# CLSFramework/gym-soccer-2d-env

Measured on AMD Instinct MI355X. Metric: env-steps/sec at 65536 parallel reach_ball envs per MI355X, higher is better.
Workload: dtype f32

## Files before the change

gym-soccer-2d-env_amd/csrc/s2d_device.h:

```cpp
#pragma once
#include <hip/hip_runtime.h>
#include <stdint.h>

#include "../../include/s2d.h"

#define S2D_DEV __device__ __forceinline__

enum { S2D_MODE_DISCRETE = 0, S2D_MODE_CONT1 = 1, S2D_MODE_TURN4 = 2 };

struct S2DHot {
  float inv_half_l, inv_half_w, half_l, half_w;
  float player_decay, ball_decay;
  float player_accel_max2, player_speed_max2, ball_speed_max2, rsum2;
  float stamina_max, stamina_inc_max, extra_stamina, stamina_capacity;
  float recover_init, recover_dec_thr_value, recover_min, recover_dec;
  float effort_init, effort_dec_thr_value, effort_min, effort_dec, effort_inc_thr_value, effort_inc;
  float dash_power_rate, max_dash_power, min_dash_power, max_dash_angle, min_dash_angle;
  float dash_angle_step, inv_dash_angle_step, side_dash_rate, back_dash_rate;
  float min_distance_to_ball, min_dist2_thr, act_scale;
  int max_steps, n_actions, auto_reset;
  uint32_t seed_lo, seed_hi, gid_lo, gid_hi;
  float max_moment, min_moment, inertia_moment, player_rand, ball_rand;
};
struct S2DRare {
// ... 515 lines not shown
    if (cmd == S2D_CMD_DASH) {
      dash_apply(p, e, c, ax, ay);
      accel = true;
    } else if (cmd == S2D_CMD_TURN) {
      cmd_turn(p, e, c.dir, NOISE, nz.tu);
    }
  }
  const float d2 = sim_move<NOISE>(p, rp, e, accel, ax, ay, nz);
  sim_tick_decay(p, e);
  update_stamina(p, e);
  return d2;
}

#define S2D_TAB_MAX 256
struct S2DTables { float ep[S2D_TAB_MAX], stamina[S2D_TAB_MAX], effort[S2D_TAB_MAX], recovery[S2D_TAB_MAX], capacity[S2D_TAB_MAX]; };
S2D_DEV void tables_build(const S2DHot& p, float recover_init, float cmd_power, int len, S2DTables& t) {
  Env e{};
  e.stamina = p.stamina_max; e.recovery = recover_init; e.effort = p.effort_init; e.capacity = p.stamina_capacity;
  update_stamina(p, e);
  for (int s = 0; s < len; ++s) {
    t.stamina[s] = e.stamina; t.effort[s] = e.effort; t.recovery[s] = e.recovery; t.capacity[s] = e.capacity;
    const float avail = e.stamina + p.extra_stamina;
    const float need = (cmd_power > avail) ? avail : cmd_power;
    const float st = e.stamina - need;
    t.ep[s] = e.effort * need;
    e.stamina = st > 0.0f ? st : 0.0f;
    update_stamina(p, e);
  }
}
template <bool NOISE>
// ... 177 lines not shown
```

gym-soccer-2d-env_amd/csrc/s2d_engine.hip:

```cpp
#include <hip/hip_runtime.h>

#include <cmath>
#include <cstdio>
#include <cstdlib>
#include <cstring>
#include <new>
#include <string>
#include <type_traits>

#include "s2d_device.h"

#include "s2d_actor_launch.h"
#include "s2d_kernels.h"

__global__ void s2d_tables_kernel(S2DHot p, const S2DRare* __restrict__ rp, S2DTables* __restrict__ t) {
  if (blockIdx.x == 0 && threadIdx.x == 0 && rp->tab_len > 0) tables_build(p, rp->recover_init, rp->tab_power, rp->tab_len, *t);
}
__global__ __launch_bounds__(kBlock) void s2d_init_kernel(S2DHot p, const S2DRare* __restrict__ rp,
                                                          float* __restrict__ S, int64_t stride, int64_t n) {
  int64_t i = (int64_t)blockIdx.x * kBlock + threadIdx.x;
  if (i >= n) return;
  S[F_STAMINA * stride + i] = p.stamina_max;
  S[F_RECOVERY * stride + i] = rp->recover_init;
  S[F_EFFORT * stride + i] = p.effort_init;
  S[F_CAPACITY * stride + i] = p.stamina_capacity;
}

template <int NK>
__global__ __launch_bounds__(kBlock) void s2d_reach_reset_kernel(S2DHot p, const S2DRare* __restrict__ rp,
                                                                 float* __restrict__ S, int64_t stride, int64_t n,
                                                                 const uint8_t* __restrict__ mask, StepOut o) {
// ... 230 lines not shown
  }
  store_obs_tile(lds[wv], ob, lane, active, o.obs + wave_first * S2D_OBS_DIM, valid);
  stats_store(srow, lane, sold, wave_first == 0 ? (unsigned long long)n * (unsigned long long)n_steps : 0ull, c1, c2, c3);
}

template <int MODE, int NK>
__global__ __launch_bounds__(kBlock) void s2d_reach_rollout_kernel(S2DHot p_sgpr, const S2DRare* __restrict__ rp,
                                                                   float* __restrict__ S, int64_t stride, int64_t n,
                                                                   int n_steps, const void* __restrict__ actions,
                                                                   int kind, RolloutOut ro, StepOut o) {
  constexpr bool NOISE = NK != S2D_NK_OFF;
  __shared__ __attribute__((aligned(16))) float lds[kWavesPerBlock][kObsTile];
  __shared__ PrepTile prep[kWavesPerBlock];
  __shared__ float4 act_lut[kWavesPerBlock][kWave];
  __shared__ float ep_lds[S2D_TAB_MAX];
  __shared__ float2 sc_lut[361];
  const S2DHot p = hot_in_vgprs(p_sgpr);
  const int lane = threadIdx.x & (kWave - 1), wv = threadIdx.x / kWave;
  const int64_t i = (int64_t)blockIdx.x * kBlock + threadIdx.x;
  const int64_t wave_first = i - lane;
  const S2DTables* const tb = tables_of(rp);
  const int tab_len = MODE != S2D_MODE_TURN4 ? rp->tab_len : 0;
  if (tab_len > 0) {
    for (int k = threadIdx.x; k < tab_len; k += kBlock) ep_lds[k] = tb->ep[k];
    for (int k = threadIdx.x; k <= 360; k += kBlock) {
      float sn, cs;
      sincos_deg((float)(k - 180), sn, cs);
      sc_lut[k] = make_float2(sn, cs);
    }
    __syncthreads();
  }
  if (wave_first >= n) return;
  const bool active = i < n;
  int64_t rows = n - wave_first; if (rows > kWave) rows = kWave;
  const int valid = (int)rows * S2D_OBS_DIM;
  const bool use_k = uses_policy_step<MODE, NOISE>(kind);
  uint32_t* const kplane = reinterpret_cast<uint32_t*>(S + F_POLICY * stride);
  Env e;
  uint32_t gl = 0, gh = 0, k0 = 0;
  if (active) {
    env_load(e, S, stride, i);
    if (use_k) k0 = kplane[i];
    uint64_t gid = (((uint64_t)p.gid_hi << 32) | p.gid_lo) + (uint64_t)i;
    gl = (uint32_t)gid; gh = (uint32_t)(gid >> 32);
// ... 104 lines not shown
#endif

#ifdef S2D_STAMPS
#define WS_STAMP_DECL uint64_t st_busy = 0, st_t0 = __builtin_amdgcn_s_memtime(); const uint64_t st_begin = st_t0, st_rt0 = __builtin_amdgcn_s_memrealtime()
#define WS_BARRIER() do { st_busy += __builtin_amdgcn_s_memtime() - st_t0; __syncthreads(); st_t0 = __builtin_amdgcn_s_memtime(); } while (0)
#define WS_STAMP_STORE() do { if (lane == 0) { float* q_ = o.terminal_obs + (wave_first + 2 * role) * S2D_OBS_DIM; \
    q_[0] = (float)st_busy; q_[1] = (float)(__builtin_amdgcn_s_memtime() - st_begin); q_[2] = (float)(st_rt0 & 0xffffff); \
    q_[3] = (float)(__builtin_amdgcn_s_memrealtime() & 0xffffff); \
    q_[4] = __int_as_float((int)__builtin_amdgcn_s_getreg((31 << 11) | 4)); q_[5] = __int_as_float((int)__builtin_amdgcn_s_getreg((31 << 11) | 20)); } } while (0)
#else
#define WS_STAMP_DECL do {} while (0)
#define WS_BARRIER() __syncthreads()
#define WS_STAMP_STORE() do {} while (0)
#endif

template <int MODE, int NK, int REC = 0>
__global__ __launch_bounds__(kWsBlock, 4) void s2d_reach_rollout_ws_kernel(S2DHot p_sgpr, const S2DRare* __restrict__ rp,
                                                                        float* __restrict__ S, int64_t stride,
                                                                        int64_t n, int n_steps,
                                                                        const void* __restrict__ actions, int kind,
                                                                        RolloutOut ro, StepOut o) {
  constexpr bool NOISE = NK != S2D_NK_OFF;
  constexpr int kActWords = NOISE ? (int)WA_WORDS : (int)WA_NPM;
  __shared__ float act[3][kActWords][kWave];
  __shared__ float snap[2][WS_WORDS][kWave];
  __shared__ float slots[kSlots][SL_WORDS][kWave];
  __shared__ __attribute__((aligned(16))) float tile[2][kObsTile];
  __shared__ float4 act_lut[kWave];
  __shared__ float ep_lds[S2D_TAB_MAX];
  __shared__ float2 sc_lut[361];
  const int lane = threadIdx.x & (kWave - 1);
  const int role = __builtin_amdgcn_readfirstlane(threadIdx.x / kWave);
  const bool nt = REC == 2 || (REC == 0 && ro.nt != 0);
  const int64_t wave_first = (int64_t)blockIdx.x * kWave;
  const int64_t i = wave_first + lane;
  const bool active = i < n;
  int64_t rows = n - wave_first; rows = rows > kWave ? kWave : rows;
  const int valid = (int)rows * S2D_OBS_DIM;
  const int n_iter = n_steps + 3;

  if (role != 1 && p_sgpr.auto_reset) {
    const uint64_t gid = (((uint64_t)p_sgpr.gid_hi << 32) | p_sgpr.gid_lo) + (uint64_t)i;
    uint32_t ep0 = 0u;
    if (active) ep0 = reinterpret_cast<const uint32_t*>(S + F_EPISODE * stride)[i];
    const int k = role == 0 ? 0 : role - 1;
    slot_fill_coop<NK>(p_sgpr, rp, slots[k], lane, (uint32_t)gid, (uint32_t)(gid >> 32), ep0 + 1u + (uint32_t)k, active,
                          reinterpret_cast<uint32_t*>(&tile[0][0]) + role * kWave);
  }

  if (role == 0) {
    if constexpr (NOISE) __builtin_amdgcn_s_setprio(S2D_NPRIO_P);
    const S2DHot& p = p_sgpr;
    const bool use_k = uses_policy_step<MODE, NOISE>(kind);
    uint32_t* const kplane = reinterpret_cast<uint32_t*>(S + F_POLICY * stride);
    uint32_t gl = 0, gh = 0, k0 = 0;
    if (active) {
      if (use_k) k0 = kplane[i];
      uint64_t gid = (((uint64_t)p.gid_hi << 32) | p.gid_lo) + (uint64_t)i;
      gl = (uint32_t)gid; gh = (uint32_t)(gid >> 32);
    }
    U4 quad{0, 0, 0, 0}, squad{0, 0, 0, 0}, nblk{0, 0, 0, 0};
    float dir = 0.0f; int cmd = 0;
    int64_t row = 0;
    const bool lut = MODE == S2D_MODE_DISCRETE && kind == S2D_ACT_RANDOM && p.n_actions <= kWave;
    if (lut && lane < p.n_actions) {
// ... 39 lines not shown
      wslot = wslot == 2 ? 0 : wslot + 1;
    };
    for (int s = 0; s < n_iter; ++s) {
      if (s == 0 && n_steps > 0) policy_step(0);
      if (s + 1 < n_steps) policy_step(s + 1);
      WS_BARRIER();
    }
    WS_STAMP_STORE();
    if (active) {
      if (use_k) kplane[i] = k0 + (uint32_t)n_steps;
      o.action_dir[i] = dir; o.action_cmd[i] = (uint8_t)cmd;
    }
  } else if (role == 1) {
    if constexpr (NOISE) __builtin_amdgcn_s_setprio(S2D_NPRIO_S);
    else __builtin_amdgcn_s_setprio(S2D_PRIO_S);
    const S2DHot p = hot_in_vgprs(p_sgpr);
    Env e;
    uint32_t gl = 0, gh = 0;
    int nth = 0, j = 0;
    if (active) {
      env_load(e, S, stride, i);
      uint64_t gid = (((uint64_t)p.gid_hi << 32) | p.gid_lo) + (uint64_t)i;
      gl = (uint32_t)gid; gh = (uint32_t)(gid >> 32);
      asm volatile("" ::"v"(e.px), "v"(e.py), "v"(e.vx), "v"(e.vy), "v"(e.body), "v"(e.stamina), "v"(e.effort),
                   "v"(e.recovery), "v"(e.capacity), "v"(e.bx), "v"(e.by), "v"(e.bvx), "v"(e.bvy),
                   "v"(e.step_number), "v"(e.cycle), "v"(e.episode));
    }
    const S2DTables* const tb = tables_of(rp);
    const int tab_len = MODE != S2D_MODE_TURN4 ? rp->tab_len : 0;
    bool fast = false;
    if (tab_len > 0) {
      bool ok = true;
      if (active) {
        const int sn = e.step_number;
        ok = sn >= 0 && sn < tab_len;
        const int q = ok ? sn : 0;
        ok = ok && e.stamina == tb->stamina[q] && e.effort == tb->effort[q] && e.recovery == tb->recovery[q] &&
             e.capacity == tb->capacity[q] && e.body == rintf(e.body) && fabsf(e.body) <= 180.0f;
      }
      fast = __ballot(active && !ok) == 0ull;
      if (fast)
        for (int k = lane; k < tab_len; k += kWave) ep_lds[k] = tb->ep[k];
    }
    if (fast || NK == S2D_NK_LATTICE) {
      for (int k = lane; k <= 360; k += kWave) {
        float sn, cs;
        sincos_deg((float)(k - 180), sn, cs);
        sc_lut[k] = make_float2(sn, cs);
      }
    }
    const ResetStamina rst = reset_stamina(p, rp);
    __syncthreads();
    WS_STAMP_DECL;
    auto loop = [&](auto fast_tag) {
      constexpr bool FAST = decltype(fast_tag)::value;
      struct ActRegs { float cmd, power, dir, rate, npm, nps, npc, nbm, nbs, nbc, ntu; };
      ActRegs cur{}, nxt{};
      float ep_cur = 0.0f; float2 sc_cur = make_float2(0.0f, 0.0f);
      int rslot = 1;
      auto fetch = [&](int slot) {
        ActRegs r{};
        if (MODE == S2D_MODE_TURN4) r.cmd = act[slot][WA_CMD][lane];
        if (!FAST) r.power = act[slot][WA_POWER][lane];
        r.dir = act[slot][WA_DIR][lane]; r.rate = act[slot][WA_RATE][lane];
// ... 174 lines not shown
        if ((fw & 0xff) && auto_reset) {
          const float (*sl)[kWave] = slots[fw >> 8];
#pragma unroll
          for (int k = 4; k < S2D_OBS_DIM; ++k) term_row[k] = ob6[k];
#pragma unroll
          for (int k = 4; k < S2D_OBS_DIM; ++k) ob6[k] = sl[SL_FIRST + k][lane];
        }
        if (REC != 0 || ro.obs) {
          float* t = &tile[b][lane * S2D_OBS_DIM];
#pragma unroll
          for (int k = 4; k < S2D_OBS_DIM; ++k) t[k] = ob6[k];
        }
      }
      WS_BARRIER();
    };
    {
      int s = 0;
      for (; s < 3 && s < n_iter; ++s) ball_iteration(s, std::false_type{});
      for (; s < n_steps + 2; ++s) ball_iteration(s, std::true_type{});
      for (; s < n_iter; ++s) ball_iteration(s, std::false_type{});
    }
    WS_STAMP_STORE();
    if (active) {
#pragma unroll
      for (int k = 4; k < S2D_OBS_DIM; ++k) o.obs[i * S2D_OBS_DIM + k] = ob6[k];
    }
  }
}

__global__ __launch_bounds__(kBlock) void s2d_world_model_kernel(const float* __restrict__ S, int64_t stride,
                                                                 int64_t n, S2DWorldModel w) {
// ... 149 lines not shown
                                     int64_t n, int n_steps, const void* actions_dev, int kind, const RolloutOut* ro,
                                     const StepOut* o, void* stream, char* name);


struct S2DEngine {
  S2DConfig cfg;
  S2DHot hot;
  S2DRare rare;
  const S2DRare* rare_dev;
  int mode;
  bool noise;
  int nk;
  int rollout_ws;
  int rollout_e;
  int rollout_nt;
  char kernel_name[160];
  int64_t n, stride;
  int device;
  char* arena;
  size_t arena_bytes;
  bool owns_arena;
  S2DBuffers buf;
  StepOut out;
  const char* last_kernel;
};

static size_t align_up(size_t v, size_t a) { return (v + a - 1) / a * a; }
static int64_t stride_for(int64_t n) { return (int64_t)align_up((size_t)n, 256); }

static_assert(sizeof(S2DRare) <= 256, "S2DTables sit 256 bytes behind S2DRare");
struct ArenaLayout {
  size_t state, obs, reward, done, result, terminal_obs, action_dir, action_cmd, stats, prep, rare, tables, total;
};
static ArenaLayout layout_for(int64_t n) {
  ArenaLayout L;
  size_t s = (size_t)stride_for(n), off = 0;
  L.state = off; off += align_up((size_t)F_COUNT * s * 4, 256);
  L.obs = off; off += align_up(s * S2D_OBS_DIM * 4, 256);
  L.reward = off; off += align_up(s * 4, 256);
  L.done = off; off += align_up(s, 256);
  L.result = off; off += align_up(s, 256);
  L.terminal_obs = off; off += align_up(s * S2D_OBS_DIM * 4, 256);
  L.action_dir = off; off += align_up(s * 4, 256);
  L.action_cmd = off; off += align_up(s, 256);
  L.stats = off; off += align_up((size_t)S2D_STATS_ROWS(n) * 8 * sizeof(unsigned long long), 256);
  L.prep = off; off += align_up((size_t)(2 * PS_WORDS + 2) * s * 4, 256);
  L.rare = off; off += align_up(sizeof(S2DRare), 256);
  L.tables = off; off += align_up(sizeof(S2DTables), 256);
  L.total = off;
  return L;
}

#define S2D_STR2(x) #x
#define S2D_STR(x) S2D_STR2(x)
S2D_API const char* s2d_version(void) { return "s2d-hip 0.4 (gfx950, abi " S2D_STR(S2D_ABI_VERSION) ")"; }
S2D_API const char* s2d_last_error(void) { return g_err.c_str(); }

S2D_API void s2d_default_config(S2DConfig* c) {
  if (!c) return;
  std::memset(c, 0, sizeof *c);
  c->abi_version = S2D_ABI_VERSION;
  c->struct_bytes = (uint32_t)sizeof(S2DConfig);
  S2DServerParams& s = c->sp;
// ... 133 lines not shown
  ArenaLayout L = layout_for(n_envs);
  S2DEngine* h = new (std::nothrow) S2DEngine();
  if (!h) return fail(S2D_ENOMEM, "host allocation failed");
  h->cfg = *cfg; h->n = n_envs; h->stride = stride_for(n_envs); h->device = device;
  h->last_kernel = "";
  dev_params_from_config(*cfg, h->hot, h->rare);
  h->mode = !cfg->task.use_continuous_action ? S2D_MODE_DISCRETE
                                             : (cfg->task.use_turning ? S2D_MODE_TURN4 : S2D_MODE_CONT1);
  h->noise = cfg->noise != 0;
  h->nk = !h->noise ? S2D_NK_OFF : (cfg->noise_model == S2D_NOISE_RCSSSERVER ? S2D_NK_SQUARE : S2D_NK_LATTICE);
  h->rollout_ws = -1;
  if (const char* v = std::getenv("S2D_ROLLOUT_WS")) h->rollout_ws = std::atoi(v) != 0 ? 1 : 0;
  h->rollout_e = 1; h->rollout_nt = -1; h->kernel_name[0] = 0;
  if (const char* v = std::getenv("S2D_ROLLOUT_E")) h->rollout_e = std::atoi(v) == 2 ? 2 : 1;
  if (const char* v = std::getenv("S2D_ROLLOUT_NT")) h->rollout_nt = std::atoi(v) != 0 ? 1 : 0;
  if (arena_dev) {
    if (arena_bytes < L.total) { delete h; return fail(S2D_ENOMEM, "arena smaller than s2d_arena_bytes()"); }
    if (reinterpret_cast<uintptr_t>(arena_dev) & 255u) { delete h; return fail(S2D_EINVAL, "arena must be 256-byte aligned"); }
    h->arena = static_cast<char*>(arena_dev); h->owns_arena = false;
  } else {
    void* p = nullptr;
    if (hipMalloc(&p, L.total) != hipSuccess) { delete h; return fail(S2D_ENOMEM, "hipMalloc of the arena failed"); }
    h->arena = static_cast<char*>(p); h->owns_arena = true;
  }
  h->arena_bytes = L.total;
  S2DBuffers& b = h->buf;
  b.n_envs = n_envs;
  float* S = reinterpret_cast<float*>(h->arena + L.state);
  float** planes[15] = {&b.player_x, &b.player_y, &b.player_vx, &b.player_vy, &b.player_body, &b.stamina,
                        &b.effort, &b.recovery, &b.stamina_capacity, &b.ball_x, &b.ball_y, &b.ball_vx,
// ... 9 lines not shown
  b.result = reinterpret_cast<uint8_t*>(h->arena + L.result);
  b.terminal_obs = reinterpret_cast<float*>(h->arena + L.terminal_obs);
  b.action_dir = reinterpret_cast<float*>(h->arena + L.action_dir);
  b.action_cmd = reinterpret_cast<uint8_t*>(h->arena + L.action_cmd);
  b.stats = reinterpret_cast<unsigned long long*>(h->arena + L.stats);
  h->out = StepOut{b.obs, b.reward, b.done, b.result, b.terminal_obs, b.action_dir, b.action_cmd, b.stats,
                   reinterpret_cast<float*>(h->arena + L.prep)};
  h->rare_dev = reinterpret_cast<const S2DRare*>(h->arena + L.rare);
  hipStream_t st = static_cast<hipStream_t>(stream);
  hipError_t e = hipMemsetAsync(h->arena, 0, L.total, st);
  if (e == hipSuccess) e = hipMemcpyAsync(h->arena + L.rare, &h->rare, sizeof(S2DRare), hipMemcpyHostToDevice, st);
  if (e == hipSuccess) {
    hipLaunchKernelGGL(s2d_init_kernel, dim3(grid_for(n_envs)), dim3(kBlock), 0, st, h->hot, h->rare_dev, S,
                       h->stride, h->n);
    hipLaunchKernelGGL(s2d_tables_kernel, dim3(1), dim3(64), 0, st, h->hot, h->rare_dev,
                       reinterpret_cast<S2DTables*>(h->arena + L.tables));
    e = hipGetLastError();
  }
  if (e != hipSuccess) {
    std::string m = std::string("arena initialisation: ") + hipGetErrorString(e);
    if (h->owns_arena) (void)hipFree(h->arena);
    delete h;
    return fail(S2D_EHIP, m);
  }
  *out = h;
  return S2D_OK;
}

S2D_API void s2d_destroy(S2DHandle h) {
  if (!h) return;
  if (h->owns_arena && h->arena) {
// ... 149 lines not shown
       s2d_reach_rollout_ws_kernel<S2D_MODE_DISCRETE, S2D_NK_SQUARE>},
      {s2d_reach_rollout_ws_kernel<S2D_MODE_CONT1, S2D_NK_OFF>, s2d_reach_rollout_ws_kernel<S2D_MODE_CONT1, S2D_NK_LATTICE>,
       s2d_reach_rollout_ws_kernel<S2D_MODE_CONT1, S2D_NK_SQUARE>},
      {s2d_reach_rollout_ws_kernel<S2D_MODE_TURN4, S2D_NK_OFF>, s2d_reach_rollout_ws_kernel<S2D_MODE_TURN4, S2D_NK_LATTICE>,
       s2d_reach_rollout_ws_kernel<S2D_MODE_TURN4, S2D_NK_SQUARE>}};
  const bool ws = h->rollout_ws < 0 ? (h->n <= kWsMaxEnvs) : (h->rollout_ws != 0);
  static const char* const mode_names[3] = {"discrete", "continuous", "turning"};
  if (ws) {
    if (h->rollout_e == 2 && h->nk != S2D_NK_SQUARE && s2d_internal_rollout2(h->mode, h->noise ? 1 : 0, &h->hot, h->rare_dev, reinterpret_cast<float*>(h->buf.player_x),
                                                   h->stride, h->n, n_steps, actions_dev, action_kind, &ro, &h->out, stream, h->kernel_name)) {
      HIP_TRY(hipGetLastError());
      h->last_kernel = h->kernel_name;
      return S2D_OK;
    }
    RollK kern_ws = table_ws[h->mode][h->nk];
    int rec = 0;
    if (h->mode == S2D_MODE_DISCRETE && !h->noise && ro.obs && ro.action && ro.reward && ro.done && ro.result) {
      kern_ws = ro.nt ? s2d_reach_rollout_ws_kernel<S2D_MODE_DISCRETE, S2D_NK_OFF, 2> : s2d_reach_rollout_ws_kernel<S2D_MODE_DISCRETE, S2D_NK_OFF, 1>;
      rec = ro.nt ? 2 : 1;
    }
    hipLaunchKernelGGL(kern_ws, dim3((unsigned)((h->n + kWave - 1) / kWave)),
                       dim3(kWsBlock), 0, static_cast<hipStream_t>(stream), h->hot, h->rare_dev,
                       reinterpret_cast<float*>(h->buf.player_x), h->stride, h->n, n_steps, actions_dev, action_kind,
                       ro, h->out);
    HIP_TRY(hipGetLastError());
    std::snprintf(h->kernel_name, sizeof h->kernel_name, "s2d_reach_rollout_ws_kernel<%s,noise=%d,rec=%d,nt=%d>", mode_names[h->mode],
                  h->nk, rec, ro.nt ? 1 : 0);
    h->last_kernel = h->kernel_name;
    return S2D_OK;
  }
  hipLaunchKernelGGL(table[h->mode][h->nk], dim3(grid_for(h->n)), dim3(kBlock), 0,
                     static_cast<hipStream_t>(stream), h->hot, h->rare_dev,
                     reinterpret_cast<float*>(h->buf.player_x), h->stride, h->n, n_steps, actions_dev, action_kind,
                     ro, h->out);
  HIP_TRY(hipGetLastError());
  std::snprintf(h->kernel_name, sizeof h->kernel_name, "s2d_reach_rollout_kernel<%s,noise=%d>", mode_names[h->mode], h->nk);
  h->last_kernel = h->kernel_name;
  return S2D_OK;
}


static int actor_fail(const char* who, const char* what) { return fail(S2D_EINVAL, std::string(who) + what); }
// ... 251 lines not shown
  HIP_TRY(hipGetLastError());
  return S2D_OK;
}

S2D_API int s2d_set_seed(S2DHandle h, uint64_t seed, void* stream) {
  if (!h) return fail(S2D_EINVAL, "NULL handle");
  DeviceGuard guard(h->device);
  const ArenaLayout L = layout_for(h->n);
  HIP_TRY(hipMemsetAsync(h->arena + L.prep + (size_t)2 * PS_WORDS * (size_t)h->stride * 4, 0, 2 * (size_t)h->stride * 4,
                         static_cast<hipStream_t>(stream)));
  h->cfg.seed = seed;
  h->hot.seed_lo = (uint32_t)seed; h->hot.seed_hi = (uint32_t)(seed >> 32);
  return S2D_OK;
}

S2D_API int s2d_debug_eval(int op, const void* in_dev, void* out_dev, int64_t n, void* stream) {
  if (!in_dev || !out_dev || n <= 0 || op < 0 || op > 15 || (op == 9 && n % 256 != 0)) return fail(S2D_EINVAL, "bad s2d_debug_eval argument");
  hipLaunchKernelGGL(s2d_debug_eval_kernel, dim3((unsigned)((n + 255) / 256)), dim3(256), 0,
                     static_cast<hipStream_t>(stream), op, static_cast<const float*>(in_dev),
                     static_cast<float*>(out_dev), n);
  HIP_TRY(hipGetLastError());
  return S2D_OK;
}
```

gym-soccer-2d-env_amd/csrc/s2d_kernels.h:

```cpp
#pragma once
#include <hip/hip_runtime.h>

#include <type_traits>

#include "s2d_device.h"
#include "s2d_net.h"

#define S2D_API extern "C" __attribute__((visibility("default")))

#ifndef S2D_BLOCK
#define S2D_BLOCK 256
#endif
static constexpr int kBlock = S2D_BLOCK;
static constexpr int kWavesPerBlock = kBlock / kWave;
static constexpr int kObsTile = kWave * S2D_OBS_DIM;
static constexpr int64_t kWsMaxEnvs = 524288;

struct StepOut {
  float* obs;
  float* reward;
  uint8_t* done;
  uint8_t* result;
  float* terminal_obs;
  float* action_dir;
// ... 170 lines not shown
    t.v[0][lane] = q.px; t.v[1][lane] = q.py; t.v[2][lane] = q.vx; t.v[3][lane] = q.vy; t.v[4][lane] = q.body;
    t.v[5][lane] = q.stamina; t.v[6][lane] = q.effort; t.v[7][lane] = q.recovery; t.v[8][lane] = q.capacity;
    t.v[9][lane] = q.bx; t.v[10][lane] = q.by; t.v[11][lane] = q.bvx; t.v[12][lane] = q.bvy;
#pragma unroll
    for (int k = 0; k < S2D_OBS_DIM; ++k) t.v[13 + k][lane] = f.o[k];
    t.v[13 + S2D_OBS_DIM][lane] = f.dist; t.v[14 + S2D_OBS_DIM][lane] = f.rel;
  }
}
S2D_DEV NextEpisode prep_take_episode(const PrepTile& t, int lane) {
  return NextEpisode{t.v[0][lane], t.v[1][lane], t.v[2][lane], t.v[3][lane], t.v[4][lane], t.v[5][lane], t.v[6][lane],
                     t.v[7][lane], t.v[8][lane], t.v[9][lane], t.v[10][lane], t.v[11][lane], t.v[12][lane]};
}

S2D_DEV const S2DTables* tables_of(const S2DRare* rp) {
  return reinterpret_cast<const S2DTables*>(reinterpret_cast<const char*>(rp) + 256);
}

template <int NK, bool FAST = false>
S2D_DEV void step_env(const S2DHot& p, const S2DRare* __restrict__ rp, Env& e, uint32_t gid_lo, uint32_t gid_hi,
                      uint32_t k, int cmd, const CmdPrep& c, ObsOut& ob, float& reward, int& done, int& result,
                      float* __restrict__ terminal_row, PrepTile* prep, int lane, bool& have_prep,
                      const float* ep_lds = nullptr, const float2* sc_lut = nullptr) {
  constexpr bool NOISE = NK != S2D_NK_OFF;
  NoiseIn nz{0.0f, 0.0f, 0.0f, 0.0f, 0.0f, 0.0f, 0.0f};
  if constexpr (NOISE) nz = noise_prepare_kind<NK>(p, gid_lo, gid_hi, k, S2D_ST_NOISE, cmd == S2D_CMD_TURN);
  float d2;
  if constexpr (FAST) {
    const float ep = ep_lds[e.step_number];
    const float2 sc = sc_lut[(int)norm_deg(e.body + c.dir) + 180];
    e.step_number += 1;
// ... 107 lines not shown
```

gym-soccer-2d-env_amd/csrc/s2d_rollout2.hip:

```cpp
#include <hip/hip_runtime.h>

#include <cstdio>

#include "s2d_kernels.h"

static constexpr int kE = 2;
static constexpr int kGroup = kWave * kE;
static constexpr int kTile2 = kGroup * S2D_OBS_DIM;

typedef float v2f32_t __attribute__((ext_vector_type(2)));
typedef int v2i32_t __attribute__((ext_vector_type(2)));

S2D_DEV float2 ld2(const float* row, int col) { return *reinterpret_cast<const float2*>(row + col); }
S2D_DEV void st2(float* row, int col, float a, float b) { *reinterpret_cast<float2*>(row + col) = make_float2(a, b); }

template <bool NT> S2D_DEV void rec2_f32(float* p, float a, float b) {
  const v2f32_t v = {a, b};
  if (NT) __builtin_nontemporal_store(v, reinterpret_cast<v2f32_t*>(p)); else *reinterpret_cast<v2f32_t*>(p) = v;
}
template <bool NT> S2D_DEV void rec2_i32(int32_t* p, int a, int b) {
  const v2i32_t v = {a, b};
  if (NT) __builtin_nontemporal_store(v, reinterpret_cast<v2i32_t*>(p)); else *reinterpret_cast<v2i32_t*>(p) = v;
}
template <bool NT> S2D_DEV void rec2_u8(uint8_t* p, int a, int b) {
// ... 49 lines not shown
#define S2D_PRIO2_B 3
#endif

template <int MODE, bool NOISE, bool NT>
__global__ __launch_bounds__(kWsBlock) void s2d_reach_rollout_ws2_kernel(S2DHot p_sgpr, const S2DRare* __restrict__ rp,
                                                                         float* __restrict__ S, int64_t stride, int64_t n,
                                                                         int n_steps, const void* __restrict__ actions, int kind,
                                                                         RolloutOut ro, StepOut o) {
  constexpr int kActWords = NOISE ? (int)WA_WORDS : (int)WA_NPM;
  __shared__ __attribute__((aligned(16))) float act[2][kActWords][kGroup];
  __shared__ __attribute__((aligned(16))) float snap[2][WS_WORDS][kGroup];
  __shared__ __attribute__((aligned(16))) float slots[kSlots][SL_WORDS][kGroup];
  __shared__ __attribute__((aligned(16))) float tile[2][kTile2];
  __shared__ float4 act_lut[kWave];
  __shared__ float ep_lds[S2D_TAB_MAX];
  __shared__ float2 sc_lut[361];
  const int lane = threadIdx.x & (kWave - 1);
  const int role = __builtin_amdgcn_readfirstlane(threadIdx.x / kWave);
  const int64_t first = (int64_t)blockIdx.x * kGroup;
  const int col = kE * lane;
  const int64_t i0 = first + col;
  const int n_iter = n_steps + 3;
  const uint64_t gid0 = (((uint64_t)p_sgpr.gid_hi << 32) | p_sgpr.gid_lo) + (uint64_t)i0;

  if (role != 1 && p_sgpr.auto_reset) {
    const uint2 ep0 = *reinterpret_cast<const uint2*>(S + F_EPISODE * stride + i0);
    const int k = role == 0 ? 0 : role - 1;
    uint32_t* const scratch = reinterpret_cast<uint32_t*>(&tile[0][0]) + role * kWave;
    const S2DRare r = *rp;
#pragma unroll
    for (int e = 0; e < kE; ++e) {
// ... 124 lines not shown
      bool ok = true;
#pragma unroll
      for (int q = 0; q < kE; ++q) {
        const int sn = e[q].step_number;
        bool okq = sn >= 0 && sn < tab_len;
        const int t = okq ? sn : 0;
        okq = okq && e[q].stamina == tb->stamina[t] && e[q].effort == tb->effort[t] && e[q].recovery == tb->recovery[t] &&
              e[q].capacity == tb->capacity[t] && e[q].body == rintf(e[q].body) && fabsf(e[q].body) <= 180.0f;
        ok = ok && okq;
      }
      fast = __ballot(!ok) == 0ull;
      if (fast)
        for (int k = lane; k < tab_len; k += kWave) ep_lds[k] = tb->ep[k];
    }
    if (fast || NOISE) {
      for (int k = lane; k <= 360; k += kWave) {
        float sn, cs;
        sincos_deg((float)(k - 180), sn, cs);
        sc_lut[k] = make_float2(sn, cs);
      }
    }
    const ResetStamina rst = reset_stamina(p, rp);
    __syncthreads();
    WS2_STAMP_DECL;
    auto loop = [&](auto fast_tag) {
      constexpr bool FAST = decltype(fast_tag)::value;
      auto simulate_iteration = [&](int s, auto steady_tag) {
        constexpr bool STEADY = decltype(steady_tag)::value;
        if (STEADY || (s >= 1 && s <= n_steps)) {
          const int b = (s - 1) & 1;
          const float2 a_dir = ld2(act[b][WA_DIR], col), a_rate = ld2(act[b][WA_RATE], col);
          float2 a_pow = make_float2(0.0f, 0.0f), a_cmd = make_float2(0.0f, 0.0f);
          if (!FAST) a_pow = ld2(act[b][WA_POWER], col);
          if (MODE == S2D_MODE_TURN4) a_cmd = ld2(act[b][WA_CMD], col);
          float2 n_pm, n_ps, n_pc, n_bm, n_bs, n_bc, n_tu = make_float2(0.0f, 0.0f);
// ... 248 lines not shown
```

gym-soccer-2d-env_amd/soccer2d_amd/_capi.py:

```python
import ctypes as C
import os

S2D_ABI_VERSION = 4
S2D_OBS_DIM = 10

S2D_OK, S2D_EINVAL, S2D_EHIP, S2D_ENOMEM, S2D_ENODEV = 0, -1, -2, -3, -4
MODE_BEFORE_KICK_OFF, MODE_TIME_OVER, MODE_PLAY_ON = 0, 1, 2
SIDE_UNKNOWN, SIDE_LEFT, SIDE_RIGHT = 0, 1, 2
RESULT_NONE, RESULT_GOAL, RESULT_OUT, RESULT_TIMEOUT = 0, 1, 2, 3
RESULT_NAMES = (None, 'Goal', 'Out', 'Timeout')
CMD_NONE, CMD_DASH, CMD_TURN, CMD_FREEZE = 0, 1, 2, -1
ACT_DISCRETE_I32, ACT_DISCRETE_I64, ACT_CONTINUOUS, ACT_TURNING, ACT_RANDOM, ACT_COMMAND = 0, 1, 2, 3, 4, 5
NOISE_LATTICE, NOISE_RCSSSERVER = 0, 1
NOISE_MODELS = {'lattice': NOISE_LATTICE, 'rcssserver': NOISE_RCSSSERVER}


class S2DLibraryError(RuntimeError):
    """libs2d_hip.so is missing / failed to load.  There is no fallback path."""


class S2DServerParams(C.Structure):
    _fields_ = [(n, C.c_double) for n in (
        'pitch_half_length', 'pitch_half_width',
        'player_size', 'player_decay', 'player_rand', 'player_speed_max', 'player_accel_max',
# ... 211 lines not shown
    ('s2d_learn_ppo', C.c_int, (C.POINTER(S2DLearnPPO), C.POINTER(S2DLearnPPOBatch), C.c_void_p)),
    ('s2d_learn_ppo_grad', C.c_int, (C.POINTER(S2DLearnPPO), C.POINTER(S2DLearnPPOBatch), C.c_void_p)),
    ('s2d_learn_sac_actor', C.c_int, (C.c_int64, C.POINTER(S2DLearnNet), C.POINTER(S2DLearnState), C.POINTER(S2DLearnNet),
                                      C.POINTER(S2DLearnNet), C.c_void_p, C.c_void_p, C.POINTER(S2DLearnSacAlpha), C.c_void_p, C.c_uint64,
                                      C.c_void_p, C.c_void_p, C.c_void_p, C.c_void_p)),
    ('s2d_learn_sac_actor_grad', C.c_int, (C.c_int64, C.POINTER(S2DLearnNet), C.POINTER(S2DLearnState), C.POINTER(S2DLearnNet),
                                           C.POINTER(S2DLearnNet), C.c_void_p, C.c_void_p, C.POINTER(S2DLearnSacAlpha), C.c_void_p,
                                           C.c_uint64, C.c_void_p, C.c_void_p, C.c_void_p, C.c_void_p)),
    ('s2d_learn_sac_workspace_bytes', C.c_size_t, (C.POINTER(S2DLearnNet), C.POINTER(S2DLearnNet), C.POINTER(S2DLearnNet), C.c_int64)),
    ('s2d_world_model', C.c_int, (C.c_void_p, C.POINTER(S2DWorldModel), C.c_void_p)),
    ('s2d_stats_reset', C.c_int, (C.c_void_p, C.c_void_p)),
    ('s2d_kernel_name', C.c_char_p, (C.c_void_p,)),
    ('s2d_validate_state', C.c_int, (C.c_void_p, C.c_void_p, C.c_void_p)),
    ('s2d_set_seed', C.c_int, (C.c_void_p, C.c_uint64, C.c_void_p)),
    ('s2d_debug_eval', C.c_int, (C.c_int, C.c_void_p, C.c_void_p, C.c_int64, C.c_void_p)),
    ('s2d_debug_net_forward', C.c_int, (C.c_int, C.c_int, C.c_int, C.c_void_p, C.c_void_p, C.c_int64, C.c_void_p, C.c_void_p,
                                        C.c_char_p, C.c_void_p)),
    ('s2d_debug_mlp_forward', C.c_int, (C.POINTER(S2DMlpNet), C.c_void_p, C.c_int64, C.c_void_p, C.c_void_p, C.c_char_p, C.c_void_p)),
    ('s2d_debug_wide_forward', C.c_int, (C.POINTER(S2DWideNet), C.c_void_p, C.c_int64, C.c_void_p, C.c_void_p, C.c_char_p, C.c_void_p)),
    ('s2d_debug_policy_head', C.c_int, (C.c_int, C.c_int, C.c_void_p, C.c_void_p, C.c_void_p, C.c_void_p, C.c_uint64, C.c_int,
                                        C.c_int64, C.c_void_p, C.c_void_p, C.c_void_p)),
)

PKG_ROOT = os.path.dirname(os.path.dirname(os.path.abspath(__file__)))
LIB_PATH = os.path.join(PKG_ROOT, 'lib', 'libs2d_hip.so')

_lib = None


def load_library(path=None):
# ... 36 lines not shown
```

include/s2d.h:

```cpp
#ifndef S2D_H_
#define S2D_H_

#include <stddef.h>
#include <stdint.h>

#ifdef __cplusplus
extern "C" {
#endif

#define S2D_ABI_VERSION 4

enum {
  S2D_OK = 0,
  S2D_EINVAL = -1,
  S2D_EHIP = -2,
  S2D_ENOMEM = -3,
  S2D_ENODEV = -4
};

enum { S2D_MODE_BEFORE_KICK_OFF = 0, S2D_MODE_TIME_OVER = 1, S2D_MODE_PLAY_ON = 2 };
enum { S2D_SIDE_UNKNOWN = 0, S2D_SIDE_LEFT = 1, S2D_SIDE_RIGHT = 2 };
enum { S2D_RESULT_NONE = 0, S2D_RESULT_GOAL = 1, S2D_RESULT_OUT = 2, S2D_RESULT_TIMEOUT = 3 };
enum { S2D_CMD_NONE = 0, S2D_CMD_DASH = 1, S2D_CMD_TURN = 2,
       S2D_CMD_FREEZE = -1  };
// ... 310 lines not shown
                        const float *obs , float *alpha ,
                        const S2DLearnSacAlpha *alpha_state , uint64_t *draws, uint64_t seed,
                        float *out_action , float *out_logp , float *out_q ,
                        void *stream);
int s2d_learn_sac_actor_grad(int64_t batch, const S2DLearnNet *actor, const S2DLearnState *actor_state, const S2DLearnNet *critic1,
                             const S2DLearnNet *critic2, const float *obs, float *alpha, const S2DLearnSacAlpha *alpha_state,
                             uint64_t *draws, uint64_t seed, float *out_action, float *out_logp, float *out_q, void *stream);
size_t s2d_learn_sac_workspace_bytes(const S2DLearnNet *actor_shape, const S2DLearnNet *critic1_shape,
                                     const S2DLearnNet *critic2_shape , int64_t max_batch);
int s2d_world_model(S2DHandle h, const S2DWorldModel *out, void *stream);
int s2d_stats_reset(S2DHandle h, void *stream);
const char *s2d_kernel_name(S2DHandle h);
int s2d_validate_state(S2DHandle h, uint32_t *counts_dev, void *stream);
int s2d_set_seed(S2DHandle h, uint64_t seed, void *stream);
int s2d_debug_eval(int op, const void *in_dev, void *out_dev, int64_t n, void *stream);
int s2d_debug_net_forward(int h1, int h2, int na, const void *params_dev, const void *obs_dev, int64_t n, void *y_dev,
                          void *greedy_dev, char *name, void *stream);
int s2d_debug_mlp_forward(const S2DMlpNet *shape, const void *obs_dev, int64_t n, void *y_dev, void *greedy_dev, char *name,
                          void *stream);
int s2d_debug_wide_forward(const S2DWideNet *shape, const void *obs_dev, int64_t n, void *y_dev, void *greedy_dev, char *name,
                           void *stream);
int s2d_debug_policy_head(int mode, int n_out, const void *y_dev, const void *log_std_dev, const void *gid_dev, const void *k_dev,
                          uint64_t seed, int deterministic, int64_t n, void *action_dev, void *logp_dev, void *stream);

#ifdef __cplusplus
}
#endif
#endif
```

Measured before the change: 100.3 billion.

## Precompute sincos table once and add specialized random-policy producer path

Builds the 361-entry sin/cos table once at init into the arena and has rollout kernels copy it into shared memory instead of recomputing sincos per block. Adds a POL=1 specialization of the warp-specialized rollout kernel for random discrete actions: the producer wave generates policy draws and writes the action LUT entries directly, and the ball/observation wave uses vectorized 16-byte stores for observation flushing. Enabled by default via rollout_pol. This adds arena space and a new kernel variant, and relies on the table offset matching the layout.

Measured after the change: 102.0 billion, median of 6. 1.02x the previous value.

```diff
diff --git a/gym-soccer-2d-env_amd/csrc/s2d_device.h b/gym-soccer-2d-env_amd/csrc/s2d_device.h
--- a/gym-soccer-2d-env_amd/csrc/s2d_device.h
+++ b/gym-soccer-2d-env_amd/csrc/s2d_device.h
@@ -553,6 +553,15 @@
 
 #define S2D_TAB_MAX 256
 struct S2DTables { float ep[S2D_TAB_MAX], stamina[S2D_TAB_MAX], effort[S2D_TAB_MAX], recovery[S2D_TAB_MAX], capacity[S2D_TAB_MAX]; };
+#define S2D_SINCOS_ENTRIES 361
+struct S2DSinCos { float2 v[S2D_SINCOS_ENTRIES]; };
+S2D_DEV void sincos_table_build(S2DSinCos& t, int first, int step) {
+  for (int k = first; k < S2D_SINCOS_ENTRIES; k += step) {
+    float sn, cs;
+    sincos_deg((float)(k - 180), sn, cs);
+    t.v[k] = make_float2(sn, cs);
+  }
+}
 S2D_DEV void tables_build(const S2DHot& p, float recover_init, float cmd_power, int len, S2DTables& t) {
   Env e{};
   e.stamina = p.stamina_max; e.recovery = recover_init; e.effort = p.effort_init; e.capacity = p.stamina_capacity;
diff --git a/gym-soccer-2d-env_amd/csrc/s2d_engine.hip b/gym-soccer-2d-env_amd/csrc/s2d_engine.hip
--- a/gym-soccer-2d-env_amd/csrc/s2d_engine.hip
+++ b/gym-soccer-2d-env_amd/csrc/s2d_engine.hip
@@ -13,8 +13,10 @@
 #include "s2d_actor_launch.h"
 #include "s2d_kernels.h"
 
-__global__ void s2d_tables_kernel(S2DHot p, const S2DRare* __restrict__ rp, S2DTables* __restrict__ t) {
-  if (blockIdx.x == 0 && threadIdx.x == 0 && rp->tab_len > 0) tables_build(p, rp->recover_init, rp->tab_power, rp->tab_len, *t);
+__global__ void s2d_tables_kernel(S2DHot p, const S2DRare* __restrict__ rp, S2DTables* __restrict__ t, S2DSinCos* __restrict__ sc) {
+  if (blockIdx.x != 0) return;
+  sincos_table_build(*sc, (int)threadIdx.x, (int)blockDim.x);
+  if (threadIdx.x == 0 && rp->tab_len > 0) tables_build(p, rp->recover_init, rp->tab_power, rp->tab_len, *t);
 }
 __global__ __launch_bounds__(kBlock) void s2d_init_kernel(S2DHot p, const S2DRare* __restrict__ rp,
                                                           float* __restrict__ S, int64_t stride, int64_t n) {
@@ -275,7 +277,7 @@
   __shared__ PrepTile prep[kWavesPerBlock];
   __shared__ float4 act_lut[kWavesPerBlock][kWave];
   __shared__ float ep_lds[S2D_TAB_MAX];
-  __shared__ float2 sc_lut[361];
+  __shared__ float2 sc_lut[S2D_SINCOS_ENTRIES];
   const S2DHot p = hot_in_vgprs(p_sgpr);
   const int lane = threadIdx.x & (kWave - 1), wv = threadIdx.x / kWave;
   const int64_t i = (int64_t)blockIdx.x * kBlock + threadIdx.x;
@@ -284,11 +286,7 @@
   const int tab_len = MODE != S2D_MODE_TURN4 ? rp->tab_len : 0;
   if (tab_len > 0) {
     for (int k = threadIdx.x; k < tab_len; k += kBlock) ep_lds[k] = tb->ep[k];
-    for (int k = threadIdx.x; k <= 360; k += kBlock) {
-      float sn, cs;
-      sincos_deg((float)(k - 180), sn, cs);
-      sc_lut[k] = make_float2(sn, cs);
-    }
+    sincos_table_copy(sc_lut, rp, (int)threadIdx.x, kBlock);
     __syncthreads();
   }
   if (wave_first >= n) return;
@@ -423,7 +421,7 @@
 #define WS_STAMP_STORE() do {} while (0)
 #endif
 
-template <int MODE, int NK, int REC = 0>
+template <int MODE, int NK, int REC = 0, int POL = 0>
 __global__ __launch_bounds__(kWsBlock, 4) void s2d_reach_rollout_ws_kernel(S2DHot p_sgpr, const S2DRare* __restrict__ rp,
                                                                         float* __restrict__ S, int64_t stride,
                                                                         int64_t n, int n_steps,
@@ -437,7 +435,7 @@
   __shared__ __attribute__((aligned(16))) float tile[2][kObsTile];
   __shared__ float4 act_lut[kWave];
   __shared__ float ep_lds[S2D_TAB_MAX];
-  __shared__ float2 sc_lut[361];
+  __shared__ float2 sc_lut[S2D_SINCOS_ENTRIES];
   const int lane = threadIdx.x & (kWave - 1);
   const int role = __builtin_amdgcn_readfirstlane(threadIdx.x / kWave);
   const bool nt = REC == 2 || (REC == 0 && ro.nt != 0);
@@ -457,7 +455,47 @@
                           reinterpret_cast<uint32_t*>(&tile[0][0]) + role * kWave);
   }
 
-  if (role == 0) {
+  if (POL == 1 && role == 0) {
+    static_assert(POL != 1 || (MODE == S2D_MODE_DISCRETE && !NOISE && REC != 0), "POL = 1: discrete actions, noise off, whole record");
+    S2DHot key{};
+    key.seed_lo = p_sgpr.seed_lo; key.seed_hi = p_sgpr.seed_hi;
+    const uint32_t n_act = (uint32_t)p_sgpr.n_actions;
+    const uint64_t gid = (((uint64_t)p_sgpr.gid_hi << 32) | p_sgpr.gid_lo) + (uint64_t)i;
+    const uint32_t gl = (uint32_t)gid, gh = (uint32_t)(gid >> 32);
+    uint32_t* const kplane = reinterpret_cast<uint32_t*>(S + F_POLICY * stride);
+    uint32_t k = 0;
+    if (active) k = kplane[i];
+    if (lane < (int)n_act) {
+      int c0; float pw, d0;
+      action_map<MODE>(p_sgpr, Action4{(float)lane, 0.0f, 0.0f, 0.0f}, 0.0f, c0, pw, d0);
+      const CmdPrep c = cmd_prepare(p_sgpr, c0, pw, d0);
+      act_lut[lane] = make_float4(c.power, c.dir, c.dir_rate, d0);
+    }
+    U4 quad{0, 0, 0, 0};
+    if ((k & 3u) != 0u) quad = policy_quad(key, gl, gh, k, S2D_ST_POLICY);
+    __syncthreads();
+    WS_STAMP_DECL;
+    int32_t* const arec = static_cast<int32_t*>(ro.action) + i;
+    float4 e4 = make_float4(0.0f, 0.0f, 0.0f, 0.0f);
+    int wslot = 0;
+    int64_t row = 0;
+    for (int t = 0; t < n_steps; ++t) {
+      if ((k & 3u) == 0u) quad = policy_quad(key, gl, gh, k, S2D_ST_POLICY);
+      const int a = rnd_below(quad_word(quad, k), n_act);
+      if (active) rec_store(arec + row, (int32_t)a, nt);
+      e4 = act_lut[a];
+      act[wslot][WA_POWER][lane] = e4.x; act[wslot][WA_DIR][lane] = e4.y; act[wslot][WA_RATE][lane] = e4.z;
+      k += 1u; row += n;
+      wslot = wslot == 2 ? 0 : wslot + 1;
+      if (t != 0) WS_BARRIER();
+    }
+    for (int s = n_steps > 1 ? n_steps - 1 : 0; s < n_iter; ++s) WS_BARRIER();
+    WS_STAMP_STORE();
+    if (active) {
+      kplane[i] = k;
+      o.action_dir[i] = e4.w; o.action_cmd[i] = (uint8_t)(n_steps > 0 ? S2D_CMD_DASH : 0);
+    }
+  } else if (role == 0) {
     if constexpr (NOISE) __builtin_amdgcn_s_setprio(S2D_NPRIO_P);
     const S2DHot& p = p_sgpr;
     const bool use_k = uses_policy_step<MODE, NOISE>(kind);
@@ -527,7 +565,8 @@
   } else if (role == 1) {
     if constexpr (NOISE) __builtin_amdgcn_s_setprio(S2D_NPRIO_S);
     else __builtin_amdgcn_s_setprio(S2D_PRIO_S);
-    const S2DHot p = hot_in_vgprs(p_sgpr);
+    S2DHot p = hot_in_vgprs(p_sgpr);
+    if constexpr (POL == 1) asm("v_mov_b32 %0, %1" : "=v"(p.max_steps) : "s"(p_sgpr.max_steps));
     Env e;
     uint32_t gl = 0, gh = 0;
     int nth = 0, j = 0;
@@ -556,11 +595,7 @@
         for (int k = lane; k < tab_len; k += kWave) ep_lds[k] = tb->ep[k];
     }
     if (fast || NK == S2D_NK_LATTICE) {
-      for (int k = lane; k <= 360; k += kWave) {
-        float sn, cs;
-        sincos_deg((float)(k - 180), sn, cs);
-        sc_lut[k] = make_float2(sn, cs);
-      }
+      sincos_table_copy(sc_lut, rp, lane, kWave);
     }
     const ResetStamina rst = reset_stamina(p, rp);
     __syncthreads();
@@ -765,7 +800,57 @@
       }
       WS_BARRIER();
     };
-    {
+    auto store16 = [&](float4* q, const float4& v) {
+      if (nt) {
+        const v4f32_t w = {v.x, v.y, v.z, v.w};
+        asm volatile("global_store_dwordx4 %0, %1, off nt\n\ts_nop 0" ::"v"(q), "v"(w) : "memory");
+      } else {
+        *q = v;
+      }
+    };
+    auto ball_iteration_vec = [&](int s, auto steady_tag) {
+      constexpr bool STEADY = decltype(steady_tag)::value;
+      const bool flush = STEADY || s >= 3;
+      const bool work = STEADY || (s >= 2 && s < n_steps + 2);
+      const int b = s & 1;
+      float4 f0 = make_float4(0.0f, 0.0f, 0.0f, 0.0f), f1 = f0, f2 = f0;
+      float bx = 0.0f, by = 0.0f, bvx = 0.0f, bvy = 0.0f; int fw = 0;
+      if (flush) {
+        const float4* t4 = reinterpret_cast<const float4*>(tile[(s - 1) & 1]);
+        f0 = t4[lane]; f1 = t4[kWave + lane]; f2 = t4[2 * kWave + (lane & 31)];
+      }
+      if (work) {
+        bx = snap[b][WS_BX][lane]; by = snap[b][WS_BY][lane];
+        bvx = snap[b][WS_BVX][lane]; bvy = snap[b][WS_BVY][lane];
+        fw = __float_as_int(snap[b][WS_FLAGS][lane]);
+      }
+      if (flush) {
+        float4* d4 = reinterpret_cast<float4*>(ro.obs + ((int64_t)(s - 3) * n + wave_first) * S2D_OBS_DIM);
+        store16(d4 + lane, f0);
+        store16(d4 + kWave + lane, f1);
+        if (lane < 32) store16(d4 + 2 * kWave + lane, f2);
+      }
+      if (work) {
+        observe_ball(p, bx, by, bvx, bvy, ob6);
+        if ((fw & 0xff) && auto_reset) {
+          const float (*sl)[kWave] = slots[fw >> 8];
+#pragma unroll
+          for (int k = 4; k < S2D_OBS_DIM; ++k) term_row[k] = ob6[k];
+#pragma unroll
+          for (int k = 4; k < S2D_OBS_DIM; ++k) ob6[k] = sl[SL_FIRST + k][lane];
+        }
+        float* t = &tile[b][lane * S2D_OBS_DIM];
+#pragma unroll
+        for (int k = 4; k < S2D_OBS_DIM; ++k) t[k] = ob6[k];
+      }
+      WS_BARRIER();
+    };
+    if (POL == 1 && obs_all_vec) {
+      int s = 0;
+      for (; s < 3 && s < n_iter; ++s) ball_iteration_vec(s, std::false_type{});
+      for (; s < n_steps + 2; ++s) ball_iteration_vec(s, std::true_type{});
+      for (; s < n_iter; ++s) ball_iteration_vec(s, std::false_type{});
+    } else {
       int s = 0;
       for (; s < 3 && s < n_iter; ++s) ball_iteration(s, std::false_type{});
       for (; s < n_steps + 2; ++s) ball_iteration(s, std::true_type{});
@@ -945,6 +1030,7 @@
   int rollout_ws;
   int rollout_e;
   int rollout_nt;
+  int rollout_pol;
   char kernel_name[160];
   int64_t n, stride;
   int device;
@@ -961,7 +1047,7 @@
 
 static_assert(sizeof(S2DRare) <= 256, "S2DTables sit 256 bytes behind S2DRare");
 struct ArenaLayout {
-  size_t state, obs, reward, done, result, terminal_obs, action_dir, action_cmd, stats, prep, rare, tables, total;
+  size_t state, obs, reward, done, result, terminal_obs, action_dir, action_cmd, stats, prep, rare, tables, sincos, total;
 };
 static ArenaLayout layout_for(int64_t n) {
   ArenaLayout L;
@@ -978,6 +1064,7 @@
   L.prep = off; off += align_up((size_t)(2 * PS_WORDS + 2) * s * 4, 256);
   L.rare = off; off += align_up(sizeof(S2DRare), 256);
   L.tables = off; off += align_up(sizeof(S2DTables), 256);
+  L.sincos = off; off += align_up(sizeof(S2DSinCos), 256);
   L.total = off;
   return L;
 }
@@ -1141,6 +1228,8 @@
   h->rollout_e = 1; h->rollout_nt = -1; h->kernel_name[0] = 0;
   if (const char* v = std::getenv("S2D_ROLLOUT_E")) h->rollout_e = std::atoi(v) == 2 ? 2 : 1;
   if (const char* v = std::getenv("S2D_ROLLOUT_NT")) h->rollout_nt = std::atoi(v) != 0 ? 1 : 0;
+  h->rollout_pol = 1;
+  if (const char* v = std::getenv("S2D_ROLLOUT_POL")) h->rollout_pol = std::atoi(v) != 0 ? 1 : 0;
   if (arena_dev) {
     if (arena_bytes < L.total) { delete h; return fail(S2D_ENOMEM, "arena smaller than s2d_arena_bytes()"); }
     if (reinterpret_cast<uintptr_t>(arena_dev) & 255u) { delete h; return fail(S2D_EINVAL, "arena must be 256-byte aligned"); }
@@ -1180,7 +1269,7 @@
     hipLaunchKernelGGL(s2d_init_kernel, dim3(grid_for(n_envs)), dim3(kBlock), 0, st, h->hot, h->rare_dev, S,
                        h->stride, h->n);
     hipLaunchKernelGGL(s2d_tables_kernel, dim3(1), dim3(64), 0, st, h->hot, h->rare_dev,
-                       reinterpret_cast<S2DTables*>(h->arena + L.tables));
+                       reinterpret_cast<S2DTables*>(h->arena + L.tables), reinterpret_cast<S2DSinCos*>(h->arena + L.sincos));
     e = hipGetLastError();
   }
   if (e != hipSuccess) {
@@ -1360,18 +1449,20 @@
       return S2D_OK;
     }
     RollK kern_ws = table_ws[h->mode][h->nk];
-    int rec = 0;
+    int rec = 0, pol = 0;
     if (h->mode == S2D_MODE_DISCRETE && !h->noise && ro.obs && ro.action && ro.reward && ro.done && ro.result) {
-      kern_ws = ro.nt ? s2d_reach_rollout_ws_kernel<S2D_MODE_DISCRETE, S2D_NK_OFF, 2> : s2d_reach_rollout_ws_kernel<S2D_MODE_DISCRETE, S2D_NK_OFF, 1>;
       rec = ro.nt ? 2 : 1;
+      pol = (h->rollout_pol != 0 && action_kind == S2D_ACT_RANDOM && h->hot.n_actions <= kWave) ? 1 : 0;
+      if (pol) kern_ws = ro.nt ? s2d_reach_rollout_ws_kernel<S2D_MODE_DISCRETE, S2D_NK_OFF, 2, 1> : s2d_reach_rollout_ws_kernel<S2D_MODE_DISCRETE, S2D_NK_OFF, 1, 1>;
+      else kern_ws = ro.nt ? s2d_reach_rollout_ws_kernel<S2D_MODE_DISCRETE, S2D_NK_OFF, 2> : s2d_reach_rollout_ws_kernel<S2D_MODE_DISCRETE, S2D_NK_OFF, 1>;
     }
     hipLaunchKernelGGL(kern_ws, dim3((unsigned)((h->n + kWave - 1) / kWave)),
                        dim3(kWsBlock), 0, static_cast<hipStream_t>(stream), h->hot, h->rare_dev,
                        reinterpret_cast<float*>(h->buf.player_x), h->stride, h->n, n_steps, actions_dev, action_kind,
                        ro, h->out);
     HIP_TRY(hipGetLastError());
-    std::snprintf(h->kernel_name, sizeof h->kernel_name, "s2d_reach_rollout_ws_kernel<%s,noise=%d,rec=%d,nt=%d>", mode_names[h->mode],
-                  h->nk, rec, ro.nt ? 1 : 0);
+    std::snprintf(h->kernel_name, sizeof h->kernel_name, "s2d_reach_rollout_ws_kernel<%s,noise=%d,rec=%d,nt=%d%s>", mode_names[h->mode],
+                  h->nk, rec, ro.nt ? 1 : 0, pol ? ",pol=1" : "");
     h->last_kernel = h->kernel_name;
     return S2D_OK;
   }
@@ -1653,6 +1744,13 @@
   return S2D_OK;
 }
 
+S2D_API int s2d_debug_sincos_table(S2DHandle h, float* out_dev, void* stream) {
+  if (!h || !out_dev) return fail(S2D_EINVAL, "NULL argument");
+  DeviceGuard guard(h->device);
+  HIP_TRY(hipMemcpyAsync(out_dev, h->arena + layout_for(h->n).sincos, sizeof(S2DSinCos), hipMemcpyDeviceToDevice, static_cast<hipStream_t>(stream)));
+  return S2D_OK;
+}
+
 S2D_API int s2d_debug_eval(int op, const void* in_dev, void* out_dev, int64_t n, void* stream) {
   if (!in_dev || !out_dev || n <= 0 || op < 0 || op > 15 || (op == 9 && n % 256 != 0)) return fail(S2D_EINVAL, "bad s2d_debug_eval argument");
   hipLaunchKernelGGL(s2d_debug_eval_kernel, dim3((unsigned)((n + 255) / 256)), dim3(256), 0,
diff --git a/gym-soccer-2d-env_amd/csrc/s2d_kernels.h b/gym-soccer-2d-env_amd/csrc/s2d_kernels.h
--- a/gym-soccer-2d-env_amd/csrc/s2d_kernels.h
+++ b/gym-soccer-2d-env_amd/csrc/s2d_kernels.h
@@ -208,6 +208,14 @@
 
 S2D_DEV const S2DTables* tables_of(const S2DRare* rp) {
   return reinterpret_cast<const S2DTables*>(reinterpret_cast<const char*>(rp) + 256);
+}
+static constexpr size_t kSinCosOffset = 256 + (sizeof(S2DTables) + 255) / 256 * 256;
+S2D_DEV const S2DSinCos* sincos_of(const S2DRare* rp) {
+  return reinterpret_cast<const S2DSinCos*>(reinterpret_cast<const char*>(rp) + kSinCosOffset);
+}
+S2D_DEV void sincos_table_copy(float2* sc_lut, const S2DRare* rp, int first, int step) {
+  const S2DSinCos* const src = sincos_of(rp);
+  for (int k = first; k < S2D_SINCOS_ENTRIES; k += step) sc_lut[k] = src->v[k];
 }
 
 template <int NK, bool FAST = false>
diff --git a/gym-soccer-2d-env_amd/csrc/s2d_rollout2.hip b/gym-soccer-2d-env_amd/csrc/s2d_rollout2.hip
--- a/gym-soccer-2d-env_amd/csrc/s2d_rollout2.hip
+++ b/gym-soccer-2d-env_amd/csrc/s2d_rollout2.hip
@@ -87,7 +87,7 @@
   __shared__ __attribute__((aligned(16))) float tile[2][kTile2];
   __shared__ float4 act_lut[kWave];
   __shared__ float ep_lds[S2D_TAB_MAX];
-  __shared__ float2 sc_lut[361];
+  __shared__ float2 sc_lut[S2D_SINCOS_ENTRIES];
   const int lane = threadIdx.x & (kWave - 1);
   const int role = __builtin_amdgcn_readfirstlane(threadIdx.x / kWave);
   const int64_t first = (int64_t)blockIdx.x * kGroup;
@@ -242,11 +242,7 @@
         for (int k = lane; k < tab_len; k += kWave) ep_lds[k] = tb->ep[k];
     }
     if (fast || NOISE) {
-      for (int k = lane; k <= 360; k += kWave) {
-        float sn, cs;
-        sincos_deg((float)(k - 180), sn, cs);
-        sc_lut[k] = make_float2(sn, cs);
-      }
+      sincos_table_copy(sc_lut, rp, lane, kWave);
     }
     const ResetStamina rst = reset_stamina(p, rp);
     __syncthreads();
diff --git a/gym-soccer-2d-env_amd/soccer2d_amd/_capi.py b/gym-soccer-2d-env_amd/soccer2d_amd/_capi.py
--- a/gym-soccer-2d-env_amd/soccer2d_amd/_capi.py
+++ b/gym-soccer-2d-env_amd/soccer2d_amd/_capi.py
@@ -249,6 +249,7 @@
     ('s2d_validate_state', C.c_int, (C.c_void_p, C.c_void_p, C.c_void_p)),
     ('s2d_set_seed', C.c_int, (C.c_void_p, C.c_uint64, C.c_void_p)),
     ('s2d_debug_eval', C.c_int, (C.c_int, C.c_void_p, C.c_void_p, C.c_int64, C.c_void_p)),
+    ('s2d_debug_sincos_table', C.c_int, (C.c_void_p, C.c_void_p, C.c_void_p)),
     ('s2d_debug_net_forward', C.c_int, (C.c_int, C.c_int, C.c_int, C.c_void_p, C.c_void_p, C.c_int64, C.c_void_p, C.c_void_p,
                                         C.c_char_p, C.c_void_p)),
     ('s2d_debug_mlp_forward', C.c_int, (C.POINTER(S2DMlpNet), C.c_void_p, C.c_int64, C.c_void_p, C.c_void_p, C.c_char_p, C.c_void_p)),
diff --git a/include/s2d.h b/include/s2d.h
--- a/include/s2d.h
+++ b/include/s2d.h
@@ -348,6 +348,7 @@
 int s2d_validate_state(S2DHandle h, uint32_t *counts_dev, void *stream);
 int s2d_set_seed(S2DHandle h, uint64_t seed, void *stream);
 int s2d_debug_eval(int op, const void *in_dev, void *out_dev, int64_t n, void *stream);
+int s2d_debug_sincos_table(S2DHandle h, float *out_dev, void *stream);
 int s2d_debug_net_forward(int h1, int h2, int na, const void *params_dev, const void *obs_dev, int64_t n, void *y_dev,
                           void *greedy_dev, char *name, void *stream);
 int s2d_debug_mlp_forward(const S2DMlpNet *shape, const void *obs_dev, int64_t n, void *y_dev, void *greedy_dev, char *name,
```
